# javahedi/SpinDynamics.jl

Measured on AMD Instinct MI355X. Metric: H|psi> matvecs/s, XXZ L=32 Sz=0, higher is better.
Workload: dtype c128

## Files before the change

spindynamics.jl_amd/csrc/kernels_apply.hip:

```cpp
#include <hip/hip_runtime.h>

#include <algorithm>
#include <type_traits>

#include "device_common.hpp"


using namespace sd_dev;

namespace {

template <int NC, int R, int BLOCK, bool FMA, bool PK, bool GEN = false, bool PACK = false>
__global__ __launch_bounds__(BLOCK, (GEN ? 5 : NC == 2 ? 4 : 5)) void k_apply_tiled(sd_dev_model dm, double *__restrict__ out_,
                                                       const double *__restrict__ psi_, int epi, sd_epi_args ea,
                                                       double *__restrict__ partials, int max_len) {
  using V = typename VT<NC>::type;
  constexpr uint32_t ES = sizeof(V);
  constexpr int WR = R * 64;
  extern __shared__ __attribute__((aligned(16))) unsigned char smem[];
  static_assert(!PACK || (PK && !GEN && R == 4 && BLOCK == 256), "packed launch: four slots of 256 rows, packed tables, chain bonds");
  constexpr int SLOT_ROWS = WR + 1;
  V *tile = reinterpret_cast<V *>(smem);
  int *lbin = reinterpret_cast<int *>(smem + (size_t)(max_len + 1) * sizeof(V));
  double *red = PACK ? reinterpret_cast<double *>(smem + (size_t)(4 * SLOT_ROWS) * sizeof(V)) : reinterpret_cast<double *>(lbin + 16 * SD_BIN_STRIDE);
  V *tile2 = reinterpret_cast<V *>(red + 32);

  if (ea.batch > 1) {
    const int64_t boff = (int64_t)blockIdx.y * ea.bstride * NC;
    psi_ += boff; out_ += boff;
    if (ea.prev) ea.prev = (const double *)ea.prev + boff;
    if (ea.phi) ea.phi = (const double *)ea.phi + boff;
    if (ea.accv) ea.accv = (double *)ea.accv + boff;
    partials += 2 * (size_t)blockIdx.y * (size_t)dm.n_singles;
    ea.negate = (ea.negate >> blockIdx.y) & 1;
  }
  const V *__restrict__ psi = reinterpret_cast<const V *>(psi_);
  const V *__restrict__ halo = reinterpret_cast<const V *>(ea.halo);
  const int tid = threadIdx.x;
  const int lane = tid & 63;
  int slot_tile = 0, team_wave = 0, team_n = 1, wv = 0;
  bool idle = false;
  if constexpr (PACK) {
    wv = __builtin_amdgcn_readfirstlane(tid >> 6);
    typedef int i4 __attribute__((ext_vector_type(4)));
    const i4 bt = *reinterpret_cast<const i4 *>(dm.blk_tiles + 4 * (size_t)blockIdx.x);
    const int st[4] = {bt.x, bt.y, bt.z, bt.w};
    slot_tile = __builtin_amdgcn_readfirstlane(wv == 0 ? st[0] : wv == 1 ? st[1] : wv == 2 ? st[2] : st[3]);
    team_n = 0;
#pragma unroll
    for (int k = 0; k < 4; ++k) {
      if (st[k] == slot_tile) ++team_n;
      if (st[k] == slot_tile && k < wv) ++team_wave;
    }
    team_wave = __builtin_amdgcn_readfirstlane(team_wave);
    team_n = __builtin_amdgcn_readfirstlane(team_n);
    idle = slot_tile < 0;
    tile += (wv - team_wave) * SLOT_ROWS;
  }
  const int i0 = (PACK ? team_wave : (tid >> 6)) * WR + lane;
  const int tix = PACK ? (idle ? 0 : slot_tile) : blockIdx.x + dm.tile_off;
  const sd_tile_rec rec = dm.single_rec[tix];
  const uint32_t P = rec.prefix;
  const int64_t base = rec.base;
  const int p = dm.p, LS = dm.LS;
  const int len = (PACK && idle) ? 0 : rec.len;
  const int nU = rec.nU;
  const int nn = dm.nn_hops;
  static_assert(!GEN || PK, "general-bond plan: packed tables only");
  const bool need_sig = GEN ? (dm.need_sig_gen != 0) : (!PK || dm.need_sig);

  V own[R];
  uint32_t sig[R];
  typedef unsigned int u4 __attribute__((ext_vector_type(4)));
  u4 pt[PK ? R : 1];
  uint32_t dg[R];
  const uint32_t off0 = (uint32_t)i0 * ES;
  {
    const __amdgpu_buffer_rsrc_t rs = make_rsrc(psi + base, (uint32_t)len * ES);
#pragma unroll
    for (int r = 0; r < R; ++r) buf_load(own[r], rs, off0 + (uint32_t)(r * 64) * ES);
    if (PK && !need_sig && !dm.diag_cache) {
      const __amdgpu_buffer_rsrc_t rg = make_rsrc(dm.suf_dg + rec.suf_off, (uint32_t)len);
#pragma unroll
      for (int r = 0; r < R; ++r) dg[r] = (uint32_t)(unsigned char)__builtin_amdgcn_raw_buffer_load_b8(rg, (uint32_t)i0 + (uint32_t)(r * 64), 0, 0);
    }
    if (need_sig) {
      const __amdgpu_buffer_rsrc_t rsig = make_rsrc(dm.suf_states + rec.suf_off, (uint32_t)len * 2u);
#pragma unroll
      for (int r = 0; r < R; ++r) sig[r] = buf_load_u16(rsig, (uint32_t)i0 * 2u + (uint32_t)(r * 64) * 2u);
    } else {
#pragma unroll
      for (int r = 0; r < R; ++r) sig[r] = 0;
    }
  }

  uint64_t fmask = 0;
  int64_t my_base = -1;
  const uint32_t bitp = p >= 1 ? ((P >> (p - 1)) & 1u) : 0u;
  if (nn > 0 && p >= 1 && !(PACK && idle)) {
    const int b = lane + 1;
    if (b <= p) my_base = dm.far_base[(size_t)tix * (size_t)p + (size_t)lane];
    fmask = __ballot(my_base >= 0);
  }
  const int st_lo = bitp ? nU : 0, st_n = bitp ? len - nU : nU;
  auto get_bond = [&](int ln) {
    FarBond fb;
    fb.base = rl64(my_base, ln); fb.J = dm.hop_J[ln];
    const bool st = ln == p - 1;
    fb.lo = st ? st_lo : 0; fb.n = st ? st_n : len;
    return fb;
  };
  constexpr bool SKIP_DEAD = NC == 1 || BLOCK == 64;
  uint32_t live = 0;
  if (SKIP_DEAD) {
#pragma unroll
    for (int r = 0; r < R; ++r)
      if ((tid & ~63) / 64 * WR + r * 64 < len) live |= 1u << r;
    live = (uint32_t)__builtin_amdgcn_readfirstlane((int)live);
  }
  auto issue = [&](const FarBond &fb, V(&v)[R]) {
    const V *__restrict__ pb = (halo && fb.base >= dm.n_local) ? halo + (fb.base - dm.n_local) : psi + fb.base;
    const __amdgpu_buffer_rsrc_t rs = make_rsrc(pb, (uint32_t)fb.n * ES);
    const uint32_t rel = off0 - (uint32_t)fb.lo * ES;
#pragma unroll
    for (int r = 0; r < R; ++r)
      if (!SKIP_DEAD || ((live >> r) & 1u)) buf_load(v[r], rs, rel + (uint32_t)(r * 64) * ES);
  };

  V va[R], vb[R];
  if (SKIP_DEAD) {
#pragma unroll
    for (int r = 0; r < R; ++r) { va[r] = V{}; vb[r] = V{}; }
  }
  FarBond fa{}, fbb{};
  uint64_t mk = fmask;
  bool have_a = false;
  auto next_lane = [&](uint64_t &m_) { const int ln = __builtin_ctzll(m_); m_ &= m_ - 1; return ln; };
  if (mk) { fa = get_bond(next_lane(mk)); issue(fa, va); have_a = true; }

  V acc[R];
  if (dm.diag_cache) {
    double dd[R];
    const __amdgpu_buffer_rsrc_t rd = make_rsrc(dm.diag_cache + base, (uint32_t)len * (uint32_t)sizeof(double));
#pragma unroll
    for (int r = 0; r < R; ++r) buf_load(dd[r], rd, (uint32_t)i0 * (uint32_t)sizeof(double) + (uint32_t)(r * 64) * (uint32_t)sizeof(double));
#pragma unroll
    for (int r = 0; r < R; ++r) acc[r] = vscale(dd[r], own[r]);
  } else if (!need_sig) {
    const int antiP = p >= 2 ? __popc((P ^ (P >> 1)) & ((1u << (p - 1)) - 1u)) : 0;
#pragma unroll
    for (int r = 0; r < R; ++r) {
      int anti = antiP + (int)(dg[r] & 15u) + (p >= 1 ? (int)(bitp ^ (dg[r] >> 4)) : 0);
      if (dm.n_zz_nn == 0) anti = 0;
      acc[r] = vscale(dm.diag_q * (double)(dm.n_zz - 2 * anti), own[r]);
    }
  } else if (dm.diag_mode == 0) {
    const DiagHead dh = diag_head(dm, P, p);
#pragma unroll
    for (int r = 0; r < R; ++r) {
      const uint64_t s = (uint64_t)P | ((uint64_t)sig[r] << p);
      acc[r] = vscale(diag_tail(dm, dh, s, p), own[r]);
    }
  } else {
#pragma unroll
    for (int r = 0; r < R; ++r) {
      const uint64_t s = (uint64_t)P | ((uint64_t)sig[r] << p);
      acc[r] = vscale(diag_of(dm, s), own[r]);
    }
  }
#pragma unroll
  for (int r = 0; r < R; ++r)
    if (i0 + r * 64 < len) tile[1 + i0 + r * 64] = own[r];
  if (PACK ? (lane == 0 && team_wave == 0) : (tid == 0)) tile[0] = V{};
  if (!PK)
    for (int k = tid; k < 16 * SD_BIN_STRIDE; k += BLOCK) {
      int n = k / SD_BIN_STRIDE, kk = k - n * SD_BIN_STRIDE;
      lbin[k] = (int)binom_g(dm, n, kk);
    }

  __syncthreads();
  while (have_a) {
    bool have_b = false;
    if (mk) { fbb = get_bond(next_lane(mk)); issue(fbb, vb); have_b = true; }
#pragma unroll
    for (int r = 0; r < R; ++r) acc[r] = accum<FMA>(acc[r], fa.J, va[r]);
    have_a = false;
    if (!have_b) break;
    if (mk) { fa = get_bond(next_lane(mk)); issue(fa, va); have_a = true; }
#pragma unroll
    for (int r = 0; r < R; ++r) acc[r] = accum<FMA>(acc[r], fbb.J, vb[r]);
  }
  if (PK && nn > 0) {
    const __amdgpu_buffer_rsrc_t rp = make_rsrc(dm.suf_part + 4 * (size_t)rec.suf_off, (uint32_t)len * 16u);
#pragma unroll
    for (int r = 0; r < R; ++r) pt[PK ? r : 0] = __builtin_amdgcn_raw_buffer_load_b128(rp, (uint32_t)i0 * 16u + (uint32_t)(r * 64) * 16u, 0, 0);
  }
  const bool wrap = !GEN && !PACK && PK && !(NC == 1 && R == 8) && nn > 0 && dm.wrap_hop == nn;
  bool wrap_on = false;
  if (wrap) {
    const uint32_t Q = P ^ (1u << dm.wrap_pb);
    const int t2q = dm.nup - __popc(Q);
    if (t2q >= 0 && t2q <= LS) {
      wrap_on = true;
      const int64_t qb = dm.addr[Q];
      const int lenq = (int)dm.binom[LS * (SD_MAX_L + 1) + t2q];
      const V *__restrict__ pbq = (halo && qb >= dm.n_local) ? halo + (qb - dm.n_local) : psi + qb;
      const __amdgpu_buffer_rsrc_t rq = make_rsrc(pbq, (uint32_t)lenq * ES);
      for (int c0 = 0; c0 < lenq; c0 += BLOCK * R) {
#pragma unroll
        for (int r = 0; r < R; ++r) buf_load(va[r], rq, off0 + (uint32_t)(c0 + r * 64) * ES);
#pragma unroll
        for (int r = 0; r < R; ++r)
          if (c0 + i0 + r * 64 < lenq) tile2[1 + c0 + i0 + r * 64] = va[r];
      }
      if (tid == 0) tile2[0] = V{};
    }
  }

  struct GBond { int64_t base; uint32_t smask; int pb; int kind; };
  auto gbond = [&](int h) {
    GBond g{0, 0u, 0, -1};
    const int bi = dm.hop_i[h] - 1, bj = dm.hop_j[h] - 1;
    const bool ip = bi < p, jp = bj < p;
    if (ip && jp) {
      if (((P >> bi) ^ (P >> bj)) & 1u) { g.kind = 0; g.base = dm.addr[P ^ (1u << bi) ^ (1u << bj)]; }
    } else if (!ip && !jp) {
      g.kind = 1; g.smask = (1u << (bi - p)) | (1u << (bj - p));
    } else {
      g.pb = ip ? bi : bj;
      g.smask = 1u << ((ip ? bj : bi) - p);
      const uint32_t Q = P ^ (1u << g.pb);
      const int t2q = dm.nup - __popc(Q);
      if (t2q >= 0 && t2q <= LS) { g.kind = 2; g.base = dm.addr[Q]; }
    }
    return g;
  };
  auto gflip = [&](const GBond &g, int r) -> bool {
    if (g.kind == 0) return true;
    if (g.kind == 1) return __popc(sig[r] & g.smask) == 1;
    if (g.kind == 2) return ((P >> g.pb) & 1u) != ((sig[r] & g.smask) ? 1u : 0u);
    return false;
  };
  auto gvalue = [&](const GBond &g, int r) -> V {
    if (g.kind == 1) return tile[1 + dm.suf_rank[sig[r] ^ g.smask]];
    const int64_t idx = g.base + (g.kind == 0 ? (int64_t)(i0 + r * 64) : (int64_t)dm.suf_rank[sig[r] ^ g.smask]);
    return (halo && idx >= dm.n_local) ? halo[idx - dm.n_local] : psi[idx];
  };
  const bool have_g = !GEN && nn < dm.n_hop;
  double gJ = 0.0;
  GBond g0{0, 0u, 0, -1};
  auto request_g0 = [&]() {
    g0 = gbond(nn);
    gJ = dm.hop_J[nn];
#pragma unroll
    for (int r = 0; r < R; ++r) va[r] = (i0 + r * 64 < len && gflip(g0, r)) ? gvalue(g0, r) : V{};
  };
  if (have_g && !PK) request_g0();
  if (nn > 0) {
    if constexpr (PK) {
      const unsigned char *tb = reinterpret_cast<const unsigned char *>(tile);
      constexpr uint32_t SH = NC == 2 ? 4 : 3;
#pragma unroll
      for (int a = 1; a <= 11; ++a) if (a <= LS - 1) {
        const double J = dm.hop_J[p + a - 1];
        const int w = (a - 1) / 3, sh = 10 * ((a - 1) % 3);
        V v[R];
#pragma unroll
        for (int r = 0; r < R; ++r) {
          const u4 q = pt[PK ? r : 0];
          const uint32_t word = w == 0 ? q.x : w == 1 ? q.y : w == 2 ? q.z : q.w;
          const uint32_t ad = ((word >> sh) & 0x3FFu) << SH;
          v[r] = *reinterpret_cast<const V *>(tb + ad);
        }
#pragma unroll
        for (int r = 0; r < R; ++r) acc[r] = accum<FMA>(acc[r], J, v[r]);
      }
    } else {
      uint32_t dw[R];
#pragma unroll
      for (int r = 0; r < R; ++r) dw[r] = sig[r] ^ (sig[r] >> 1);
      for (int a = 1; a <= LS - 1; ++a) {
        const double J = dm.hop_J[p + a - 1];
        const int *brow = lbin + (LS - a - 1) * SD_BIN_STRIDE;
        int d[R];
#pragma unroll
        for (int r = 0; r < R; ++r) d[r] = brow[__popc(sig[r] >> (a + 1))];
        V v[R];
#pragma unroll
        for (int r = 0; r < R; ++r) {
          const bool up = (sig[r] >> (a - 1)) & 1u;
          const bool fl = (dw[r] >> (a - 1)) & 1u;
          const int ip = (i0 + r * 64) + (up ? d[r] : -d[r]);
          v[r] = tile[fl ? ip + 1 : 0];
        }
#pragma unroll
        for (int r = 0; r < R; ++r) acc[r] = accum<FMA>(acc[r], J, v[r]);
      }
    }
  }
  if constexpr (GEN) {
    constexpr uint32_t SH = NC == 2 ? 4 : 3;
    const unsigned char *tb = reinterpret_cast<const unsigned char *>(tile);
    const unsigned char *tb2 = reinterpret_cast<const unsigned char *>(tile2);
    uint32_t ptw[R];
    int cur_word = -1;
    auto gissue = [&](int64_t gbase, V(&v)[R]) {
      const V *__restrict__ pbp = (halo && gbase >= dm.n_local) ? halo + (gbase - dm.n_local) : psi + gbase;
      const __amdgpu_buffer_rsrc_t rs = make_rsrc(pbp, (uint32_t)len * ES);
#pragma unroll
      for (int r = 0; r < R; ++r) buf_load(v[r], rs, off0 + (uint32_t)(r * 64) * ES);
    };
    for (int hb = 0; hb < dm.n_gen; hb += 64) {
      const int nb = dm.n_gen - hb < 64 ? dm.n_gen - hb : 64;
      int64_t base_k = -1;
      sd_gbond gl{-1, 0u, 0, 0, 0.0};
      if (lane < nb) {
        gl = dm.gen[hb + lane];
        if (gl.kind == 0 && __popc(P & gl.pmask) == 1) base_k = dm.addr[P ^ gl.pmask];
      }
      uint64_t todo = __ballot(base_k >= 0);
      int in_a = -1;
      if (todo) { in_a = next_lane(todo); gissue(rl64(base_k, in_a), va); }
#pragma nounroll
      for (int k = 0; k < nb; ++k) {
        sd_gbond gb;
        gb.kind = rl(gl.kind, k); gb.pmask = (uint32_t)rl((int)gl.pmask, k); gb.slot = rl(gl.slot, k); gb.pb = rl(gl.pb, k);
        gb.J = rld(gl.J, k);
        if (gb.kind == 0) {
          if (k == in_a) {
#pragma unroll
            for (int r = 0; r < R; ++r) acc[r] = accum<false>(acc[r], gb.J, va[r]);
            in_a = -1;
            if (todo) { in_a = next_lane(todo); gissue(rl64(base_k, in_a), va); }
          }
        } else if (gb.kind == 1) {
          const int wi = gb.slot / 3, sh = 10 * (gb.slot - 3 * wi);
          if (wi != cur_word) {
            cur_word = wi;
            const int chunk = wi >> 2;
            const __amdgpu_buffer_rsrc_t rp2 = make_rsrc(dm.gen_ss_part + 4 * ((size_t)chunk * (size_t)dm.n_suf_rows + (size_t)rec.suf_off), (uint32_t)len * 16u);
            const uint32_t wo = (uint32_t)(wi & 3) * 4u;
#pragma unroll
            for (int r = 0; r < R; ++r) ptw[r] = (uint32_t)__builtin_amdgcn_raw_buffer_load_b32(rp2, (uint32_t)i0 * 16u + (uint32_t)(r * 64) * 16u + wo, 0, 0);
          }
          V v[R];
#pragma unroll
          for (int r = 0; r < R; ++r) v[r] = *reinterpret_cast<const V *>(tb + ((((ptw[r] >> sh) & 0x3FFu)) << SH));
#pragma unroll
          for (int r = 0; r < R; ++r) acc[r] = accum<false>(acc[r], gb.J, v[r]);
        } else if (gb.kind == 2) {
          const uint32_t Q = P ^ gb.pmask;
          const int t2q = dm.nup - __popc(Q);
          const bool ok = t2q >= 0 && t2q <= LS;
          __syncthreads();
          if (ok) {
            const int64_t qb = dm.addr[Q];
            const int lenq = (int)dm.binom[LS * (SD_MAX_L + 1) + t2q];
            const V *__restrict__ pbq = (halo && qb >= dm.n_local) ? halo + (qb - dm.n_local) : psi + qb;
            const __amdgpu_buffer_rsrc_t rq = make_rsrc(pbq, (uint32_t)lenq * ES);
            for (int c0 = 0; c0 < lenq; c0 += BLOCK * R) {
              V tmp[R];
#pragma unroll
              for (int r = 0; r < R; ++r) buf_load(tmp[r], rq, off0 + (uint32_t)(c0 + r * 64) * ES);
#pragma unroll
              for (int r = 0; r < R; ++r)
                if (c0 + i0 + r * 64 < lenq) tile2[1 + c0 + i0 + r * 64] = tmp[r];
            }
            if (tid == 0) tile2[0] = V{};
          }
          __syncthreads();
          if (ok) {
            const __amdgpu_buffer_rsrc_t rm = make_rsrc(dm.mix_part + ((size_t)gb.slot * (size_t)dm.n_suf_rows + (size_t)rec.suf_off), (uint32_t)len * 2u);
            const uint32_t bpb = (P >> gb.pb) & 1u;
            uint32_t w16[R];
#pragma unroll
            for (int r = 0; r < R; ++r) w16[r] = buf_load_u16(rm, (uint32_t)i0 * 2u + (uint32_t)(r * 64) * 2u);
#pragma unroll
            for (int r = 0; r < R; ++r) {
              const bool has = (w16[r] >> 15) != bpb;
              const uint32_t ad = has ? ((w16[r] & 0x3FFu) << SH) : 0u;
              acc[r] = accum<false>(acc[r], gb.J, *reinterpret_cast<const V *>(tb2 + ad));
            }
          }
        }
      }
    }
  }
  if (wrap) {
    __syncthreads();
    if (wrap_on) {
      const double Jw = dm.hop_J[nn];
      const uint32_t bpb = (P >> dm.wrap_pb) & 1u;
      const unsigned char *tb2 = reinterpret_cast<const unsigned char *>(tile2);
      constexpr uint32_t SH = NC == 2 ? 4 : 3;
#pragma unroll
      for (int r = 0; r < R; ++r) {
        const uint32_t w3 = pt[PK ? r : 0].w;
        const bool has = ((w3 >> 30) & 1u) != bpb;
        const uint32_t ad = has ? (((w3 >> 20) & 0x3FFu) << SH) : 0u;
        acc[r] = accum<false>(acc[r], Jw, *reinterpret_cast<const V *>(tb2 + ad));
      }
    }
  }
  if (have_g) {
    if (!wrap) {
      if (PK) request_g0();
#pragma unroll
      for (int r = 0; r < R; ++r)
        if (gflip(g0, r)) acc[r] = accum<false>(acc[r], gJ, va[r]);
    }
    for (int h = nn + 1; h < dm.n_hop; ++h) {
      const GBond g = gbond(h);
      if (g.kind < 0) continue;
      const double J = dm.hop_J[h];
#pragma unroll
      for (int r = 0; r < R; ++r)
        if (i0 + r * 64 < len && gflip(g, r)) acc[r] = accum<false>(acc[r], J, gvalue(g, r));
    }
  }

  EpiSums sums{0.0, 0.0};
#pragma unroll
  for (int r = 0; r < R; ++r) {
    const int i = i0 + r * 64;
    if (i < len) epilogue<NC>(epi, ea, base + i, acc[r], tile[1 + i], out_, sums);
  }
  if (epi_has_sums(epi)) {
    double a = sums.s0, b = sums.s1;
    if constexpr (PACK) {
      for (int off = 32; off > 0; off >>= 1) {
        a += __shfl_down(a, off, 64);
        b += __shfl_down(b, off, 64);
      }
      if (lane == 0) { red[2 * wv] = a; red[2 * wv + 1] = b; }
      __syncthreads();
      if (lane == 0 && team_wave == 0 && !idle) {
        double x = 0.0, y = 0.0;
        for (int w = 0; w < team_n; ++w) { x += red[2 * (wv + w)]; y += red[2 * (wv + w) + 1]; }
        partials[2 * (size_t)tix] = x; partials[2 * (size_t)tix + 1] = y;
      }
    } else {
      block_reduce2(a, b, red);
      if (tid == 0) { partials[2 * (size_t)tix] = a; partials[2 * (size_t)tix + 1] = b; }
    }
  }
}

template <int NC, bool FMA>
__global__ __launch_bounds__(256, 4) void k_apply_fulltile(sd_dev_model dm, double *__restrict__ out_,
                                                        const double *__restrict__ psi_, int epi, sd_epi_args ea,
                                                        double *__restrict__ partials) {
  using V = typename VT<NC>::type;
  constexpr uint32_t ES = sizeof(V);
  constexpr int R = 4, BLOCK = 256;
  extern __shared__ __attribute__((aligned(16))) unsigned char smem[];
  const int LF = dm.full_ls, TL = 1 << LF;
  V *tile = reinterpret_cast<V *>(smem);
  double *red = reinterpret_cast<double *>(smem + (size_t)(TL + 1) * sizeof(V));
  const V *__restrict__ psi = reinterpret_cast<const V *>(psi_);
  const V *__restrict__ halo = reinterpret_cast<const V *>(ea.halo);
  const int tid = threadIdx.x, lane = tid & 63;
  uint32_t T = blockIdx.x;
  if (gridDim.x >= 512 && (gridDim.x & 255u) == 0) {
    const uint32_t x = T & 7u, j = T >> 3, g = j >> 5, i = j & 31u;
    T = (g << 8) + (x << 5) + i;
  }
  const int64_t base = (int64_t)T << LF;
  const uint32_t Tg = T + (uint32_t)(dm.row_lo >> LF);
  const int64_t gbase = (int64_t)Tg << LF;
  const int nn = dm.nn_hops;

  V own[R];
  uint32_t ioff[R];
  {
    const __amdgpu_buffer_rsrc_t rs = make_rsrc(psi + base, (uint32_t)TL * ES);
#pragma unroll
    for (int r = 0; r < R; ++r) { ioff[r] = (uint32_t)(tid + r * BLOCK) * ES; buf_load(own[r], rs, ioff[r]); }
  }
  uint64_t fmask = 0;
  int64_t my_base = 0;
  double my_J = 0.0;
  int my_lo = 0, my_n = TL;
  if (nn > 0) {
    const int a = LF + lane;
    bool fl = false;
    if (a <= dm.L - 1) {
      if (lane == 0) {
        const int t = (int)(T & 1u);
        my_lo = (1 - t) * (TL / 2); my_n = TL / 2;
        my_base = ((int64_t)(T ^ 1u) << LF) + (TL / 2 - my_lo);
        fl = true;
      } else {
        const int b = a - LF - 1;
        fl = ((Tg >> b) ^ (Tg >> (b + 1))) & 1u;
        const uint32_t Tp = Tg ^ (3u << b);
        const int tb = dm.L - LF - dm.fs_dbits;
        const uint32_t q = Tp >> tb;
        const int64_t at_peer = (int64_t)(Tp & ((1u << tb) - 1u)) << LF;
        my_base = at_peer;
        if (q != (Tg >> tb)) {
          int64_t ho = 0, plo = 0;
#pragma unroll
          for (int q2 = 0; q2 < SD_FS_MAX_RANKS; ++q2)
            if ((uint32_t)q2 == q) { ho = dm.fs_halo_off[q2]; plo = dm.fs_peer_lo[q2]; }
          my_base = dm.n_local + ho + at_peer - plo;
        }
      }
      my_J = dm.hop_J[a - 1];
    }
    fmask = __ballot(fl);
  }
  auto get_bond = [&](int ln) {
    FarBond fb;
    fb.base = rl64(my_base, ln); fb.J = rld(my_J, ln);
    fb.lo = rl(my_lo, ln); fb.n = rl(my_n, ln);
    return fb;
  };
  auto issue = [&](const FarBond &fb, V(&v)[R]) {
    const V *__restrict__ pb = (halo && fb.base >= dm.n_local) ? halo + (fb.base - dm.n_local) : psi + fb.base;
    const __amdgpu_buffer_rsrc_t rs = make_rsrc(pb, (uint32_t)fb.n * ES);
    const uint32_t lo_b = (uint32_t)fb.lo * ES;
#pragma unroll
    for (int r = 0; r < R; ++r) buf_load(v[r], rs, ioff[r] - lo_b);
  };
  V va[R], vb[R];
  FarBond fa{}, fbb{};
  uint64_t mk = fmask;
  bool have_a = false;
  auto next_lane = [&](uint64_t &m_) { const int ln = __builtin_ctzll(m_); m_ &= m_ - 1; return ln; };
  if (mk) { fa = get_bond(next_lane(mk)); issue(fa, va); have_a = true; }

  V acc[R];
#pragma unroll
  for (int r = 0; r < R; ++r) {
    acc[r] = vscale(diag_of(dm, (uint64_t)gbase + (uint64_t)(tid + r * BLOCK)), own[r]);
    tile[tid + r * BLOCK] = own[r];
  }
  if (tid == 0) tile[TL] = V{};
  __syncthreads();

  const int n_in = nn > 0 ? LF - 1 : 0;
  for (int a = 1; a <= n_in; ++a) {
    const double J = dm.hop_J[a - 1];
    V v[R];
#pragma unroll
    for (int r = 0; r < R; ++r) {
      const int i = tid + r * BLOCK;
      const bool fl = ((i >> (a - 1)) ^ (i >> a)) & 1;
      v[r] = tile[fl ? (i ^ (3 << (a - 1))) : TL];
    }
#pragma unroll
    for (int r = 0; r < R; ++r) acc[r] = accum<FMA>(acc[r], J, v[r]);
  }
  while (have_a) {
    bool have_b = false;
    if (mk) { fbb = get_bond(next_lane(mk)); issue(fbb, vb); have_b = true; }
#pragma unroll
    for (int r = 0; r < R; ++r) acc[r] = accum<FMA>(acc[r], fa.J, va[r]);
    have_a = false;
    if (!have_b) break;
    if (mk) { fa = get_bond(next_lane(mk)); issue(fa, va); have_a = true; }
#pragma unroll
    for (int r = 0; r < R; ++r) acc[r] = accum<FMA>(acc[r], fbb.J, vb[r]);
  }
  for (int h = nn; h < dm.n_hop; ++h) {
    const int bi = dm.hop_i[h] - 1, bj = dm.hop_j[h] - 1;
    const double J = dm.hop_J[h];
#pragma unroll
    for (int r = 0; r < R; ++r) {
      const uint64_t s = (uint64_t)gbase + (uint64_t)(tid + r * BLOCK);
      if (((s >> bi) ^ (s >> bj)) & 1) acc[r] = accum<false>(acc[r], J, psi[s ^ ((uint64_t)1 << bi) ^ ((uint64_t)1 << bj)]);
    }
  }
  EpiSums sums{0.0, 0.0};
#pragma unroll
  for (int r = 0; r < R; ++r) {
    const int i = tid + r * BLOCK;
    epilogue<NC>(epi, ea, base + i, acc[r], tile[i], out_, sums);
  }
  if (epi_has_sums(epi)) {
    double a = sums.s0, b = sums.s1;
    block_reduce2(a, b, red);
    if (tid == 0) { partials[2 * (size_t)blockIdx.x] = a; partials[2 * (size_t)blockIdx.x + 1] = b; }
  }
}

template <int NC>
__global__ __launch_bounds__(256) void k_apply_generic(sd_dev_model dm, double *__restrict__ out_,
                                                       const double *__restrict__ psi_, int epi, sd_epi_args ea,
                                                       double *__restrict__ partials) {
  using V = typename VT<NC>::type;
  __shared__ double red[32];
  __shared__ int64_t lb[64 * 64];
  const V *__restrict__ psi = reinterpret_cast<const V *>(psi_);
  const bool full = dm.nup < 0;
  const int L = dm.L;
  if (!full) {
    for (int i = threadIdx.x; i < 64 * 64; i += blockDim.x) {
      const int n = i >> 6, k = i & 63;
      lb[i] = (n <= L && k <= n) ? dm.binom[n * (SD_MAX_L + 1) + k] : 0;
    }
    __syncthreads();
  }
  auto bl = [&](int n, int k) -> int64_t { return (k < 0 || k > n) ? 0 : lb[(n << 6) + k]; };
  auto unrank_l = [&](int64_t idx) {
    uint64_t s = 0;
    int r = dm.nup;
    for (int k = 1; k <= L && r > 0; ++k) {
      const int64_t c = bl(L - k, r - 1);
      if (idx < c) { s |= (uint64_t)1 << (k - 1); --r; }
      else idx -= c;
    }
    return s;
  };
  auto rank_l = [&](uint64_t s) {
    int64_t idx = 0;
    int r = dm.nup;
    for (int k = 1; k <= L && r > 0; ++k) {
      if ((s >> (k - 1)) & 1) --r;
      else idx += bl(L - k, r - 1);
    }
    return idx;
  };
  const int nn = full ? 0 : dm.nn_hops;
  EpiSums sums{0.0, 0.0};
  const int64_t stride = (int64_t)gridDim.x * blockDim.x;
  for (int64_t idx = (int64_t)blockIdx.x * blockDim.x + threadIdx.x; idx < dm.N; idx += stride) {
    const uint64_t s = full ? (uint64_t)idx : unrank_l(idx);
    const V own = psi[idx];
    V acc = vscale(diag_of(dm, s), own);
    for (int b = 1; b <= nn; ++b)
      if (((s >> (b - 1)) ^ (s >> b)) & 1) {
        const int64_t d = lb[((L - b - 1) << 6) + __popcll(s >> (b + 1))];
        const int64_t nidx = ((s >> (b - 1)) & 1) ? idx + d : idx - d;
        acc = vadd_mul(acc, dm.hop_J[b - 1], psi[nidx]);
      }
    for (int h = nn; h < dm.n_hop; ++h) {
      const int bi = dm.hop_i[h] - 1, bj = dm.hop_j[h] - 1;
      if (((s >> bi) ^ (s >> bj)) & 1) {
        const uint64_t s2 = s ^ ((uint64_t)1 << bi) ^ ((uint64_t)1 << bj);
        const int64_t nidx = full ? (int64_t)s2 : rank_l(s2);
        acc = vadd_mul(acc, dm.hop_J[h], psi[nidx]);
      }
    }
    epilogue<NC>(epi, ea, idx, acc, own, out_, sums);
  }
  if (epi_has_sums(epi)) {
    double a = sums.s0, b = sums.s1;
    block_reduce2(a, b, red);
    if (threadIdx.x == 0) { partials[2 * (size_t)blockIdx.x] = a; partials[2 * (size_t)blockIdx.x + 1] = b; }
  }
}

template <int NC, int LPT>
__global__ __launch_bounds__(256) void k_apply_short(sd_dev_model dm, double *__restrict__ out_, const double *__restrict__ psi_, int epi,
                                                     sd_epi_args ea, double *__restrict__ partials, int first, int count) {
  using V = typename VT<NC>::type;
  __shared__ int64_t lb[64 * 64];
  if (ea.batch > 1) {
    const int64_t boff = (int64_t)blockIdx.y * ea.bstride * NC;
    psi_ += boff; out_ += boff;
    if (ea.prev) ea.prev = (const double *)ea.prev + boff;
    if (ea.phi) ea.phi = (const double *)ea.phi + boff;
    if (ea.accv) ea.accv = (double *)ea.accv + boff;
    partials += 2 * (size_t)blockIdx.y * (size_t)dm.n_singles;
    ea.negate = (ea.negate >> blockIdx.y) & 1;
  }
  const V *__restrict__ psi = reinterpret_cast<const V *>(psi_);
  const int L = dm.L, p = dm.p;
  for (int i = threadIdx.x; i < 64 * 64; i += blockDim.x) {
    const int n = i >> 6, k = i & 63;
    lb[i] = (n <= L && k <= n) ? dm.binom[n * (SD_MAX_L + 1) + k] : 0;
  }
  __syncthreads();
  auto bl = [&](int n, int k) -> int64_t { return (k < 0 || k > n) ? 0 : lb[(n << 6) + k]; };
  auto rank_l = [&](uint64_t s) {
    int64_t idx = 0;
    int r = dm.nup;
    for (int k = 1; k <= L && r > 0; ++k) {
      if ((s >> (k - 1)) & 1) --r;
      else idx += bl(L - k, r - 1);
    }
    return idx;
  };
  constexpr int TPB = 256 / LPT;
  const int i = threadIdx.x % LPT;
  const int nn = dm.nn_hops;
  const int sweeps = (count + (int)gridDim.x * TPB - 1) / ((int)gridDim.x * TPB);
  for (int sw = 0; sw < sweeps; ++sw) {
    const int g = (sw * (int)gridDim.x + (int)blockIdx.x) * TPB + (int)threadIdx.x / LPT;
    const bool have_tile = g < count;
    const int tix = first + (have_tile ? g : 0);
    const sd_tile_rec rec = dm.single_rec[tix];
    EpiSums sums{0.0, 0.0};
    if (have_tile && i < rec.len) {
      const int64_t idx = rec.base + i;
      const uint64_t s = (uint64_t)rec.prefix | ((uint64_t)dm.suf_states[rec.suf_off + i] << p);
      const V own = psi[idx];
      V acc = vscale(dm.diag_cache ? dm.diag_cache[idx] : diag_of(dm, s), own);
      for (int b = 1; b <= nn; ++b)
        if (((s >> (b - 1)) ^ (s >> b)) & 1) {
          const int64_t d = lb[((L - b - 1) << 6) + __popcll(s >> (b + 1))];
          const int64_t nidx = ((s >> (b - 1)) & 1) ? idx + d : idx - d;
          acc = vadd_mul(acc, dm.hop_J[b - 1], psi[nidx]);
        }
      for (int h = nn; h < dm.n_hop; ++h) {
        const int bi = dm.hop_i[h] - 1, bj = dm.hop_j[h] - 1;
        if (((s >> bi) ^ (s >> bj)) & 1) {
          const uint64_t s2 = s ^ ((uint64_t)1 << bi) ^ ((uint64_t)1 << bj);
          acc = vadd_mul(acc, dm.hop_J[h], psi[rank_l(s2)]);
        }
      }
      epilogue<NC>(epi, ea, idx, acc, own, out_, sums);
    }
    if (epi_has_sums(epi)) {
      double a = sums.s0, b = sums.s1;
      if (LPT > 1)
        for (int off = LPT / 2; off > 0; off >>= 1) {
          a += __shfl_down(a, off, LPT);
          b += __shfl_down(b, off, LPT);
        }
      if (have_tile && i == 0) { partials[2 * (size_t)tix] = a; partials[2 * (size_t)tix + 1] = b; }
    }
  }
}

template <int NC>
__global__ __launch_bounds__(256) void k_epilogue_only(int epi, sd_epi_args ea, int64_t n, double *out_,
                                                       const double *hpsi_, const double *__restrict__ psi_,
                                                       double *__restrict__ partials) {
  using V = typename VT<NC>::type;
  __shared__ double red[32];
  const V *hpsi = reinterpret_cast<const V *>(hpsi_);
  const V *__restrict__ psi = reinterpret_cast<const V *>(psi_);
  EpiSums sums{0.0, 0.0};
  const int64_t stride = (int64_t)gridDim.x * blockDim.x;
  for (int64_t i = (int64_t)blockIdx.x * blockDim.x + threadIdx.x; i < n; i += stride) {
    const V acc = hpsi[i], own = psi[i];
    epilogue<NC>(epi, ea, i, acc, own, out_, sums);
  }
  if (epi_has_sums(epi)) {
    double a = sums.s0, b = sums.s1;
    block_reduce2(a, b, red);
    if (threadIdx.x == 0) { partials[2 * (size_t)blockIdx.x] = a; partials[2 * (size_t)blockIdx.x + 1] = b; }
  }
}

__global__ __launch_bounds__(1024) void k_reduce_pairs(const double *__restrict__ partials, int64_t n,
                                                       double *__restrict__ scalars, int64_t dstride) {
  __shared__ double red[32];
  partials += 2 * (size_t)blockIdx.x * (size_t)n;
  scalars += (size_t)blockIdx.x * (size_t)dstride;
  double a = 0.0, b = 0.0;
  for (int64_t i = threadIdx.x; i < n; i += blockDim.x) { a += partials[2 * i]; b += partials[2 * i + 1]; }
  block_reduce2(a, b, red);
  if (threadIdx.x == 0) { scalars[0] = a; scalars[1] = b; }
}

__global__ __launch_bounds__(256) void k_reduce_pairs_stage(const double *__restrict__ partials, int64_t n, int64_t chunk,
                                                            double *__restrict__ stage) {
  __shared__ double red[32];
  const int64_t lo = (int64_t)blockIdx.x * chunk, hi = lo + chunk < n ? lo + chunk : n;
  const double2 *__restrict__ p2 = reinterpret_cast<const double2 *>(partials);
  double a = 0.0, b = 0.0;
  for (int64_t i = lo + threadIdx.x; i < hi; i += blockDim.x) { const double2 v = p2[i]; a += v.x; b += v.y; }
  block_reduce2(a, b, red);
  if (threadIdx.x == 0) { stage[2 * blockIdx.x] = a; stage[2 * blockIdx.x + 1] = b; }
}

}
int sd_reduce_pairs(sd_ctx *ctx, int64_t n, double *dst) {
  if (!dst) dst = ctx->d_scalars;
  const double *src = ctx->d_partials;
  if (n > 16384) {
    double *stage = ctx->d_partials + 2 * n;
    const int64_t chunk = (n + SD_RED_STAGE_BLOCKS - 1) / SD_RED_STAGE_BLOCKS;
    hipLaunchKernelGGL(k_reduce_pairs_stage, dim3(SD_RED_STAGE_BLOCKS), dim3(256), 0, ctx->stream, src, n, chunk, stage);
    SD_HIP(ctx, hipGetLastError());
    src = stage; n = SD_RED_STAGE_BLOCKS;
  }
  hipLaunchKernelGGL(k_reduce_pairs, dim3(1), dim3(1024), 0, ctx->stream, src, n, dst, (int64_t)0);
  SD_HIP(ctx, hipGetLastError());
  return SD_OK;
}
int sd_reduce_pairs_batched(sd_ctx *ctx, int64_t n, int batch, double *dst, int64_t dstride) {
  if (!dst || n > 16384 || batch < 1) return sd_set_err(ctx, SD_EINTERNAL, "bad batched reduction");
  hipLaunchKernelGGL(k_reduce_pairs, dim3((unsigned)batch), dim3(1024), 0, ctx->stream, ctx->d_partials, n, dst, dstride);
  SD_HIP(ctx, hipGetLastError());
  return SD_OK;
}
int sd_launch_epilogue_only(sd_ctx *ctx, int dtype, int64_t n, void *out, const void *hpsi, const void *psi, int epi,
                            const sd_epi_args &ea_in) {
  const bool sums = (epi == SD_EPI_DOT || epi == SD_EPI_KPM || epi == SD_EPI_RESCALE_DOT);
  sd_epi_args ea = ea_in;
  ea.stream_hint = 0;
  if (n <= 0) {
    if (sums) SD_HIP(ctx, hipMemsetAsync(ea.sums_dst ? ea.sums_dst : ctx->d_scalars, 0, 2 * sizeof(double), ctx->stream));
    return SD_OK;
  }
  const int64_t nb = std::min<int64_t>((n + 255) / 256, 4096);
  if (sums) { int rc = sd_ensure_partials(ctx, 2 * (size_t)nb + 2 * SD_RED_STAGE_BLOCKS); if (rc) return rc; }
  if (dtype == SD_C128)
    hipLaunchKernelGGL(k_epilogue_only<2>, dim3((unsigned)nb), dim3(256), 0, ctx->stream, epi, ea, n, (double *)out,
                       (const double *)hpsi, (const double *)psi, ctx->d_partials);
  else
    hipLaunchKernelGGL(k_epilogue_only<1>, dim3((unsigned)nb), dim3(256), 0, ctx->stream, epi, ea, n, (double *)out,
                       (const double *)hpsi, (const double *)psi, ctx->d_partials);
  SD_HIP(ctx, hipGetLastError());
  if (sums) return sd_reduce_pairs(ctx, nb, ea.sums_dst);
  return SD_OK;
}
namespace {

template <int NC, int R, int BLOCK, bool FMA, bool PK, bool GEN = false, bool PACK = false>
int launch_tiled_cfg(sd_ctx *ctx, const sd_dev_model &dm, int nt, size_t shmem, double *out, const double *psi, int epi,
                     const sd_epi_args &ea, int max_len) {
  void (*kern)(sd_dev_model, double *, const double *, int, sd_epi_args, double *, int) = k_apply_tiled<NC, R, BLOCK, FMA, PK, GEN, PACK>;
  if (shmem > 48 * 1024)
    SD_HIP(ctx, hipFuncSetAttribute((const void *)kern, hipFuncAttributeMaxDynamicSharedMemorySize, (int)shmem));
  hipLaunchKernelGGL(kern, dim3(nt, ea.batch > 1 ? ea.batch : 1), dim3(BLOCK), shmem, ctx->stream, dm, out, psi, epi, ea, ctx->d_partials, max_len);
  SD_HIP(ctx, hipGetLastError());
  return SD_OK;
}

template <int NC, bool FMA>
int launch_tiled(sd_ctx *ctx, const sd_dev_model &dm, int nt, int cls, size_t shmem, double *out, const double *psi, int epi,
                 const sd_epi_args &ea, int max_len) {
  constexpr int R = 4;
  if ((64 << cls) * R < max_len) return sd_set_err(ctx, SD_EINTERNAL, "tile longer than its workgroup can hold");
  if (!dm.suf_part) {
    switch (cls) {
      case 3: return launch_tiled_cfg<NC, R, 512, FMA, false>(ctx, dm, nt, shmem, out, psi, epi, ea, max_len);
      case 4: return launch_tiled_cfg<NC, R, 1024, FMA, false>(ctx, dm, nt, shmem, out, psi, epi, ea, max_len);
    }
    return sd_set_err(ctx, SD_EINTERNAL, "bad tile length class for a plan without the packed partner table");
  }
  if (dm.n_gen > 0)
    switch (cls) {
      case 0: return launch_tiled_cfg<NC, R, 64, FMA, true, true>(ctx, dm, nt, shmem, out, psi, epi, ea, max_len);
      case 1: return launch_tiled_cfg<NC, R, 128, FMA, true, true>(ctx, dm, nt, shmem, out, psi, epi, ea, max_len);
      case 2: return launch_tiled_cfg<NC, R, 256, FMA, true, true>(ctx, dm, nt, shmem, out, psi, epi, ea, max_len);
      default: return sd_set_err(ctx, SD_EINTERNAL, "bad tile length class");
    }
  constexpr bool F8 = NC == 1;
  switch (cls) {
    case 0: return launch_tiled_cfg<NC, R, 64, FMA, true>(ctx, dm, nt, shmem, out, psi, epi, ea, max_len);
    case 1: return launch_tiled_cfg<NC, F8 ? 8 : R, F8 ? 64 : 128, FMA, true>(ctx, dm, nt, shmem, out, psi, epi, ea, max_len);
    case 2: return launch_tiled_cfg<NC, F8 ? 8 : R, F8 ? 128 : 256, FMA, true>(ctx, dm, nt, shmem, out, psi, epi, ea, max_len);
  }
  return sd_set_err(ctx, SD_EINTERNAL, "bad tile length class");
}

}

int sd_launch_apply(sd_ctx *ctx, const sd_model *m, int dtype, void *out, const void *psi, int epi,
                    const sd_epi_args &ea_in, int part) {
  if (!m->dev_ready) return sd_set_err(ctx, SD_EARG, "model has no device tables (created without a context)");
  if (dtype != SD_F64 && dtype != SD_C128) return sd_set_err(ctx, SD_EARG, "dtype must be SD_F64 or SD_C128");
  const bool sums = (epi == SD_EPI_DOT || epi == SD_EPI_KPM || epi == SD_EPI_RESCALE_DOT);
  sd_dev_model dm = m->dm;
  sd_epi_args ea = ea_in;
  ea.stream_hint = 3;
  if (dm.n_local == 0) {
    if (sums) SD_HIP(ctx, hipMemsetAsync(ea.sums_dst ? ea.sums_dst : ctx->d_scalars, 0, 2 * sizeof(double), ctx->stream));
    return SD_OK;
  }
  if (ea.no_reduce && (m->p < 0 || part != 0)) return sd_set_err(ctx, SD_EINTERNAL, "unreduced sums: whole tiled plans only");
  if (ea.batch > 1 && (m->p < 0 || m->nranks != 1 || part != 0 || dm.n_singles > 16384 || (sums && !ea.sums_dst && !ea.no_reduce)))
    return sd_set_err(ctx, SD_EINTERNAL, "batched apply: unsharded tiled plans with at most 16384 tiles only");
  if (m->p >= 0) {
    int nt = dm.n_singles;
    if (part == 1) nt = dm.n_interior;
    else if (part == 2) nt = dm.n_singles - dm.n_interior;
    if (sums) { int rc = sd_ensure_partials(ctx, 2 * (size_t)dm.n_singles * (size_t)std::max(ea.batch, 1) + 2 * SD_RED_STAGE_BLOCKS); if (rc) return rc; }
    const int max_len = m->max_tile_len;
    const size_t esz = dtype == SD_C128 ? 16 : 8;
    int rc = SD_OK;
    if (nt > 0) {
      const bool packed = part == 0 && dtype == SD_C128 && dm.n_blk > 0;
      if (packed) {
        const size_t shmem = (size_t)4 * 257 * esz + 32 * sizeof(double) + 16;
        rc = m->hop_pow2 ? launch_tiled_cfg<2, 4, 256, true, true, false, true>(ctx, dm, dm.n_blk, shmem, (double *)out, (const double *)psi, epi, ea, 1024)
                         : launch_tiled_cfg<2, 4, 256, false, true, false, true>(ctx, dm, dm.n_blk, shmem, (double *)out, (const double *)psi, epi, ea, 1024);
      }
      const int s0 = part == 2 ? SD_N_LEN_CLASS : 0, s1 = packed ? s0 : part == 1 ? SD_N_LEN_CLASS : 2 * SD_N_LEN_CLASS;
      for (int sg = s0; sg < s1 && rc == SD_OK; ++sg) {
        const int cnt = m->seg_off[sg + 1] - m->seg_off[sg];
        if (cnt <= 0) continue;
        const int cls = m->seg_cls[sg];
        const int seg_max = std::min(max_len, (64 << cls) * 4);
        size_t shmem = (size_t)(seg_max + 1) * esz + 16 * SD_BIN_STRIDE * sizeof(int) + 32 * sizeof(double) + 16;
        if ((dm.wrap_hop >= 0 && dm.wrap_hop == dm.nn_hops) || dm.n_gen_mixed > 0) shmem += (size_t)(m->max_tile_len_all + 1) * esz;
        dm.tile_off = m->seg_off[sg];
        if (dtype == SD_C128)
          rc = m->hop_pow2 ? launch_tiled<2, true>(ctx, dm, cnt, cls, shmem, (double *)out, (const double *)psi, epi, ea, seg_max)
                           : launch_tiled<2, false>(ctx, dm, cnt, cls, shmem, (double *)out, (const double *)psi, epi, ea, seg_max);
        else
          rc = m->hop_pow2 ? launch_tiled<1, true>(ctx, dm, cnt, cls, shmem, (double *)out, (const double *)psi, epi, ea, seg_max)
                           : launch_tiled<1, false>(ctx, dm, cnt, cls, shmem, (double *)out, (const double *)psi, epi, ea, seg_max);
      }
      if (rc) return rc;
      if (dm.n_short > 0 && part == 0) {
        const unsigned by = ea.batch > 1 ? (unsigned)ea.batch : 1u;
        auto blocks = [](int tiles, int per_block) { return (unsigned)std::min(4096, std::max(1, (tiles + per_block - 1) / per_block)); };
        const int n16 = dm.n_short_multi, n1 = dm.n_short - dm.n_short_multi;
        if (n16 > 0) {
          if (dtype == SD_C128) hipLaunchKernelGGL((k_apply_short<2, 16>), dim3(blocks(n16, 16), by), dim3(256), 0, ctx->stream, dm, (double *)out, (const double *)psi, epi, ea, ctx->d_partials, dm.short_off, n16);
          else hipLaunchKernelGGL((k_apply_short<1, 16>), dim3(blocks(n16, 16), by), dim3(256), 0, ctx->stream, dm, (double *)out, (const double *)psi, epi, ea, ctx->d_partials, dm.short_off, n16);
        }
        if (n1 > 0) {
          if (dtype == SD_C128) hipLaunchKernelGGL((k_apply_short<2, 1>), dim3(blocks(n1, 256), by), dim3(256), 0, ctx->stream, dm, (double *)out, (const double *)psi, epi, ea, ctx->d_partials, dm.short_off + n16, n1);
          else hipLaunchKernelGGL((k_apply_short<1, 1>), dim3(blocks(n1, 256), by), dim3(256), 0, ctx->stream, dm, (double *)out, (const double *)psi, epi, ea, ctx->d_partials, dm.short_off + n16, n1);
        }
        SD_HIP(ctx, hipGetLastError());
      }
    }
    if (sums && part != 1 && !ea.no_reduce) {
      int rc2 = ea.batch > 1 ? sd_reduce_pairs_batched(ctx, (int64_t)dm.n_singles, ea.batch, ea.sums_dst, ea.sums_bstride)
                             : sd_reduce_pairs(ctx, (int64_t)dm.n_singles, ea.sums_dst);
      if (rc2) return rc2;
    }
  } else if (m->full_ls > 0) {
    if (part == 1) return SD_OK;
    const int64_t nb = dm.n_local >> m->full_ls;
    if (sums) { int rc = sd_ensure_partials(ctx, 2 * (size_t)nb + 2 * SD_RED_STAGE_BLOCKS); if (rc) return rc; }
    const size_t esz = dtype == SD_C128 ? 16 : 8;
    const size_t shmem = (((size_t)1 << m->full_ls) + 1) * esz + 32 * sizeof(double) + 16;
    void (*kf)(sd_dev_model, double *, const double *, int, sd_epi_args, double *) =
        dtype == SD_C128 ? (m->hop_pow2 ? k_apply_fulltile<2, true> : k_apply_fulltile<2, false>)
                         : (m->hop_pow2 ? k_apply_fulltile<1, true> : k_apply_fulltile<1, false>);
    hipLaunchKernelGGL(kf, dim3((unsigned)nb), dim3(256), shmem, ctx->stream, dm, (double *)out, (const double *)psi, epi, ea,
                       ctx->d_partials);
    SD_HIP(ctx, hipGetLastError());
    if (sums) {
      int rc2 = sd_reduce_pairs(ctx, (int64_t)nb, ea.sums_dst);
      if (rc2) return rc2;
    }
  } else {
    int64_t nb = (dm.N + 255) / 256;
    if (nb > 8192) nb = 8192;
    if (sums) { int rc = sd_ensure_partials(ctx, 2 * (size_t)nb + 2 * SD_RED_STAGE_BLOCKS); if (rc) return rc; }
    if (dtype == SD_C128)
      hipLaunchKernelGGL(k_apply_generic<2>, dim3((unsigned)nb), dim3(256), 0, ctx->stream, dm, (double *)out,
                         (const double *)psi, epi, ea, ctx->d_partials);
    else
      hipLaunchKernelGGL(k_apply_generic<1>, dim3((unsigned)nb), dim3(256), 0, ctx->stream, dm, (double *)out,
                         (const double *)psi, epi, ea, ctx->d_partials);
    SD_HIP(ctx, hipGetLastError());
    if (sums) {
      int rc2 = sd_reduce_pairs(ctx, (int64_t)nb, ea.sums_dst);
      if (rc2) return rc2;
    }
  }
  return SD_OK;
}
```

Measured before the change: 93.95.

## Use fixed-depth ring of far-bond loads and cap packed-launch occupancy via LDS padding

For the packed c128 launch, the alternating two-buffer far-bond loop becomes a fixed-trip ring of D register sets (default 2). Bonds past the end of the mask get zero coupling and zero-length buffer descriptors, so the loop runs without data-dependent branches. It also inflates the dynamic shared-memory request so that about SD_PACK_WGS_PER_CU workgroups fit per CU, limiting occupancy on purpose. The risks are wasted predicated loads on padding slots and lower occupancy, which may not hide latency as well as the original launch.

After: 97.40 (median of 6 runs). +3.7%, better.

```diff
diff --git a/spindynamics.jl_amd/csrc/kernels_apply.hip b/spindynamics.jl_amd/csrc/kernels_apply.hip
--- a/spindynamics.jl_amd/csrc/kernels_apply.hip
+++ b/spindynamics.jl_amd/csrc/kernels_apply.hip
@@ -10,6 +10,14 @@
 
 namespace {
 
+#ifndef SD_PACK_RING
+#define SD_PACK_RING 2
+#endif
+#ifndef SD_PACK_WGS_PER_CU
+#define SD_PACK_WGS_PER_CU 4
+#endif
+static_assert(SD_PACK_RING >= 2 && SD_PACK_RING <= 4, "ring depth of the packed launch: 2..4 register sets");
+static_assert(SD_PACK_WGS_PER_CU >= 2 && SD_PACK_WGS_PER_CU <= 6, "workgroups per CU of the packed launch: 2..6");
 template <int NC, int R, int BLOCK, bool FMA, bool PK, bool GEN = false, bool PACK = false>
 __global__ __launch_bounds__(BLOCK, (GEN ? 5 : NC == 2 ? 4 : 5)) void k_apply_tiled(sd_dev_model dm, double *__restrict__ out_,
                                                        const double *__restrict__ psi_, int epi, sd_epi_args ea,
@@ -136,7 +144,36 @@
   uint64_t mk = fmask;
   bool have_a = false;
   auto next_lane = [&](uint64_t &m_) { const int ln = __builtin_ctzll(m_); m_ &= m_ - 1; return ln; };
-  if (mk) { fa = get_bond(next_lane(mk)); issue(fa, va); have_a = true; }
+  constexpr int D = PACK ? SD_PACK_RING : 2;
+  V vx[D > 2 ? D - 2 : 1][R];
+  FarBond fr[D];
+  int ring_iters = 0;
+  auto ring_next = [&]() {
+    FarBond fb;
+    const bool e = mk == 0;
+    const int ln = e ? 0 : __builtin_ctzll(mk);
+    mk &= mk - 1;
+    fb.base = e ? 0 : rl64(my_base, ln);
+    fb.J = 0.0;
+    if (!e) fb.J = dm.hop_J[ln];
+    const bool st = ln == p - 1;
+    fb.lo = st ? st_lo : 0; fb.n = e ? 0 : st ? st_n : len;
+    return fb;
+  };
+  auto ring_issue = [&](const FarBond &fb, V(&v)[R]) {
+    const __amdgpu_buffer_rsrc_t rs = make_rsrc(psi + fb.base, (uint32_t)fb.n * ES);
+    const uint32_t rel = off0 - (uint32_t)fb.lo * ES;
+#pragma unroll
+    for (int r = 0; r < R; ++r) buf_load(v[r], rs, rel + (uint32_t)(r * 64) * ES);
+  };
+  if constexpr (PACK) {
+    const int nf = __popcll(fmask);
+    ring_iters = nf > D ? (nf + D - 1) / D : 1;
+    fr[0] = ring_next();
+    ring_issue(fr[0], va);
+  } else {
+    if (mk) { fa = get_bond(next_lane(mk)); issue(fa, va); have_a = true; }
+  }
 
   V acc[R];
   if (dm.diag_cache) {
@@ -179,16 +216,38 @@
     }
 
   __syncthreads();
-  while (have_a) {
-    bool have_b = false;
-    if (mk) { fbb = get_bond(next_lane(mk)); issue(fbb, vb); have_b = true; }
-#pragma unroll
-    for (int r = 0; r < R; ++r) acc[r] = accum<FMA>(acc[r], fa.J, va[r]);
-    have_a = false;
-    if (!have_b) break;
-    if (mk) { fa = get_bond(next_lane(mk)); issue(fa, va); have_a = true; }
-#pragma unroll
-    for (int r = 0; r < R; ++r) acc[r] = accum<FMA>(acc[r], fbb.J, vb[r]);
+  if constexpr (PACK) {
+#pragma unroll
+    for (int k = 1; k < D; ++k) { fr[k] = ring_next(); ring_issue(fr[k], k == 1 ? vb : vx[k > 2 ? k - 2 : 0]); }
+#pragma unroll
+    for (int k = 0; k < D; ++k) {
+      V(&v)[R] = k == 0 ? va : k == 1 ? vb : vx[k > 2 ? k - 2 : 0];
+#pragma unroll
+      for (int r = 0; r < R; ++r) acc[r] = accum<FMA>(acc[r], fr[k].J, v[r]);
+    }
+#pragma nounroll
+    for (int it = 1; it < ring_iters; ++it) {
+#pragma unroll
+      for (int k = 0; k < D; ++k) { fr[k] = ring_next(); ring_issue(fr[k], k == 0 ? va : k == 1 ? vb : vx[k > 2 ? k - 2 : 0]); }
+#pragma unroll
+      for (int k = 0; k < D; ++k) {
+        V(&v)[R] = k == 0 ? va : k == 1 ? vb : vx[k > 2 ? k - 2 : 0];
+#pragma unroll
+        for (int r = 0; r < R; ++r) acc[r] = accum<FMA>(acc[r], fr[k].J, v[r]);
+      }
+    }
+  } else {
+    while (have_a) {
+      bool have_b = false;
+      if (mk) { fbb = get_bond(next_lane(mk)); issue(fbb, vb); have_b = true; }
+#pragma unroll
+      for (int r = 0; r < R; ++r) acc[r] = accum<FMA>(acc[r], fa.J, va[r]);
+      have_a = false;
+      if (!have_b) break;
+      if (mk) { fa = get_bond(next_lane(mk)); issue(fa, va); have_a = true; }
+#pragma unroll
+      for (int r = 0; r < R; ++r) acc[r] = accum<FMA>(acc[r], fbb.J, vb[r]);
+    }
   }
   if (PK && nn > 0) {
     const __amdgpu_buffer_rsrc_t rp = make_rsrc(dm.suf_part + 4 * (size_t)rec.suf_off, (uint32_t)len * 16u);
@@ -879,7 +938,9 @@
     if (nt > 0) {
       const bool packed = part == 0 && dtype == SD_C128 && dm.n_blk > 0;
       if (packed) {
-        const size_t shmem = (size_t)4 * 257 * esz + 32 * sizeof(double) + 16;
+        constexpr size_t LDS_CU = 160 * 1024, WGS = SD_PACK_WGS_PER_CU;
+        const size_t need = (size_t)4 * 257 * esz + 32 * sizeof(double) + 16;
+        const size_t shmem = WGS >= 6 ? need : std::max(need, ((LDS_CU / WGS + LDS_CU / (WGS + 1)) / 2) & ~(size_t)255);
         rc = m->hop_pow2 ? launch_tiled_cfg<2, 4, 256, true, true, false, true>(ctx, dm, dm.n_blk, shmem, (double *)out, (const double *)psi, epi, ea, 1024)
                          : launch_tiled_cfg<2, 4, 256, false, true, false, true>(ctx, dm, dm.n_blk, shmem, (double *)out, (const double *)psi, epi, ea, 1024);
       }
```
